# darcamo/pyphysim

Measured on AMD Instinct MI355X. Metric: Monte Carlo realizations/sec (whole node) + SER abs-error vs ref, higher is better.
Workload: dtype f64

## Files before the change

pyphysim_amd/csrc/capi.hip:

```cpp
#include <cmath>
#include <cstdarg>

#include "common.hpp"
#include "modem.hpp"

namespace mcle {

static thread_local char g_err[512] = "";

void set_error(const char* fmt, ...) {
    va_list ap;
    va_start(ap, fmt);
    vsnprintf(g_err, sizeof(g_err), fmt, ap);
    va_end(ap);
}

}

using namespace mcle;

int mcle_ctx::bind() const {
    MCLE_HIP(hipSetDevice(device));
    return MCLE_OK;
}
// ... 155 lines not shown
    if (ctx->ev1) (void)hipEventDestroy(ctx->ev1);
    if (ctx->ev_probe0) (void)hipEventDestroy(ctx->ev_probe0);
    if (ctx->ev_probe1) (void)hipEventDestroy(ctx->ev_probe1);
    if (ctx->own_stream && ctx->stream) (void)hipStreamDestroy(ctx->stream);
    delete ctx;
    return MCLE_OK;
}

int mcle_ctx_set_stream(mcle_ctx* ctx, void* hip_stream) {
    MCLE_REQUIRE(ctx != nullptr, "null context");
    MCLE_HIP(hipSetDevice(ctx->device));
    MCLE_HIP(hipStreamSynchronize(ctx->stream));
    if (ctx->own_stream && ctx->stream) MCLE_HIP(hipStreamDestroy(ctx->stream));
    if (hip_stream) {
        ctx->stream = (hipStream_t)hip_stream;
        ctx->own_stream = false;
    } else {
        MCLE_HIP(hipStreamCreateWithFlags(&ctx->stream, hipStreamNonBlocking));
        ctx->own_stream = true;
    }
    return MCLE_OK;
}

int mcle_ctx_get_stream(mcle_ctx* ctx, void** hip_stream) {
    MCLE_REQUIRE(ctx != nullptr && hip_stream != nullptr, "null argument");
    *hip_stream = (void*)ctx->stream;
    return MCLE_OK;
}

int mcle_ctx_set_option(mcle_ctx* ctx, int option, long long value) {
    MCLE_REQUIRE(ctx != nullptr, "null context");
    MCLE_REQUIRE(option >= 0 && option < MCLE_OPT_COUNT, "unknown option %d", option);
    bool ok = false;
    switch (option) {
        case MCLE_OPT_NO_MFMA: case MCLE_OPT_SINGLE_TDL: case MCLE_OPT_JAKES_DIRECT: case MCLE_OPT_F64_GENERIC: case MCLE_OPT_BD_RUNTIME_SOLVE: case MCLE_OPT_DEMOD_NOCERT: case MCLE_OPT_F32_MFMA: case MCLE_OPT_WALK_LEGACY: case MCLE_OPT_STAGED_GENERIC: case MCLE_OPT_CODEBOOK_NO_PACK: ok = value == 0 || value == 1; break;
        case MCLE_OPT_TDL_KERNEL: ok = value >= 0 && value <= 4; break;
#ifdef MCLE_EXPERIMENTS
        case MCLE_OPT_MIMO_TDL_KERNEL: ok = value >= 0 && value <= 255; break;
#else
        case MCLE_OPT_MIMO_TDL_KERNEL: ok = value >= 0 && value <= 2; break;
#endif
#ifdef MCLE_EXPERIMENTS
        case MCLE_OPT_F64_VARIANT: ok = value >= 0 && value <= 2047; break;
#else
        case MCLE_OPT_F64_VARIANT:
            MCLE_REQUIRE(value == 0, "option MCLE_OPT_F64_VARIANT: the timing-bound variants are compiled with -DMCLE_EXPERIMENTS only");
            ok = true;
            break;
#endif
        case MCLE_OPT_MFMA_VARIANT: ok = value == 0 || value == 36 || value == 32 || value == 30 || value == 21; break;
        case MCLE_OPT_GRID_OVERSUB: ok = value >= 0 && value <= 64; break;
        case MCLE_OPT_FLAT_WGS_PER_CU: ok = value >= 0 && value <= 4096; break;
        case MCLE_OPT_TDL_MFMA_WAVES: ok = value == 0 || value == 2 || value == 3 || value == 32; break;
        case MCLE_OPT_F64_THREADS: ok = value == 0 || (value >= 256 && value <= 266) || value == 512 || value == 1024; break;
    }
    MCLE_REQUIRE(ok, "option %d: value %lld out of range", option, value);
    ctx->opt[option] = value;
    return MCLE_OK;
}

int mcle_ctx_trim_scratch(mcle_ctx* ctx) {
    MCLE_REQUIRE(ctx != nullptr, "null context");
    MCLE_HIP(hipSetDevice(ctx->device));
    MCLE_HIP(hipStreamSynchronize(ctx->stream));
    if (ctx->d_scratch) MCLE_HIP(hipFree(ctx->d_scratch));
    ctx->d_scratch = nullptr;
    ctx->scratch_bytes = 0;
    return MCLE_OK;
}

int mcle_ctx_get_option(mcle_ctx* ctx, int option, long long* value) {
    MCLE_REQUIRE(ctx != nullptr && value != nullptr, "null argument");
    MCLE_REQUIRE(option >= 0 && option < MCLE_OPT_COUNT, "unknown option %d", option);
    *value = ctx->opt[option];
    return MCLE_OK;
}

int mcle_ctx_sync(mcle_ctx* ctx) {
    MCLE_REQUIRE(ctx != nullptr, "null context");
    MCLE_HIP(hipSetDevice(ctx->device));
    MCLE_HIP(hipStreamSynchronize(ctx->stream));
    return MCLE_OK;
}

int mcle_ctx_device_info(mcle_ctx* ctx, int* n_cu, int* lds_bytes, char* name, int name_len) {
    MCLE_REQUIRE(ctx != nullptr, "null context");
    if (n_cu) *n_cu = ctx->n_cu;
    if (lds_bytes) *lds_bytes = ctx->lds_bytes;
    if (name && name_len > 0) {
        std::strncpy(name, ctx->name.c_str(), name_len - 1);
        name[name_len - 1] = 0;
    }
    return MCLE_OK;
}

int mcle_ctx_last_kernel(mcle_ctx* ctx, char* name, int len) {
    MCLE_REQUIRE(ctx != nullptr && name != nullptr && len > 0, "null argument");
    std::strncpy(name, ctx->last_kernel, len - 1);
    name[len - 1] = 0;
    return MCLE_OK;
}

int mcle_malloc(mcle_ctx* ctx, size_t bytes, void** d_ptr) {
    MCLE_REQUIRE(ctx != nullptr && d_ptr != nullptr, "null argument");
    MCLE_HIP(hipSetDevice(ctx->device));
    *d_ptr = nullptr;
    if (bytes == 0) return MCLE_OK;
// ... 283 lines not shown
```

pyphysim_amd/csrc/pipeline_mimo_planar.hip:

```cpp
#include <type_traits>
#include <utility>

#include "fft.hpp"
#include "fft_r16.hpp"
#include "mimo.hpp"
#include "modem.hpp"
#include "philox.hpp"
#include "totals.hpp"
#include "pipe_common.hpp"
#include "mimo_planar_common.hpp"

namespace mcle {

template <typename T, int N, int NT, int NR, int AH, int WPS, int VAR = 0>
__global__ __launch_bounds__((N / 4) * (NR / AH), WPS) void k_run_mimo_ofdm_planar(MimoParams pp, ModemParams<T> mp, uint64_t seed,
                                                                     uint64_t first, uint64_t count,
                                                                     const cx<T>* __restrict__ g_tw,
                                                                     const cx<T>* __restrict__ g_recs,
                                                                     mcle_counters* counters,
                                                                     uint32_t* __restrict__ sym_out,
                                                                     uint32_t* __restrict__ bit_out) {
    using SH = F64Shape<N>;
    static_assert(NT >= 1 && NT <= NR && NR % AH == 0 && N >= 256, "geometry");
    constexpr int kRec = d64_rec<NT, NR>(), NB = SH::NB, N4 = SH::N4;
// ... 406 lines not shown
        hipLaunchKernelGGL((k_mimo_filters_planar<T, N, NT, NR>), dim3((unsigned)((n + 63) / 64)), dim3(64), 0, ctx->stream, pp, seed,
                           first + off, n, (cx<T>*)recs);
        MCLE_LAUNCH_CHECK();
        const unsigned grid = (unsigned)oversubscribed_grid(ctx, resident, n, flush_min_units(8, sizeof(T) == 4 ? 25600 : 12800, (uint64_t)N * NR), 16);
        hipLaunchKernelGGL(kern, dim3(grid), dim3(TB), lds, ctx->stream, pp, mp, seed, first + off, n,
                           (const cx<T>*)tw, (const cx<T>*)recs, d_counters, d_sym ? d_sym + off : nullptr,
                           d_bit ? d_bit + off : nullptr);
        MCLE_LAUNCH_CHECK();
    }
    return MCLE_OK;
}

#ifndef MCLE_PLANAR_F32_WPS_PLUS
#define MCLE_PLANAR_F32_WPS_PLUS 2
#endif
template <typename T> constexpr int planar_wps(int n, int nt, int nr, int w64) {
    if (sizeof(T) == 4 && w64 <= 3 && ((n == 256 && !(nt == 4 && nr == 4)) || (n == 512 && nr == 2))) return w64 + MCLE_PLANAR_F32_WPS_PLUS;
#ifndef MCLE_PLANAR_F64_256_WPS3
#define MCLE_PLANAR_F64_256_WPS3 0
#endif
    if (MCLE_PLANAR_F64_256_WPS3 && sizeof(T) == 8 && n == 256 && nr <= 3 && w64 == 2) return 3;
    return w64;
}

int run_mimo_ofdm_qw(mcle_ctx* ctx, const mcle_mimo_ofdm_cfg* cfg, uint64_t seed, uint64_t first, uint64_t count,
                     mcle_counters* d_counters, uint32_t* d_sym, uint32_t* d_bit);

int run_mimo_ofdm_fw(mcle_ctx* ctx, int dtype, const mcle_mimo_ofdm_cfg* cfg, uint64_t seed, uint64_t first, uint64_t count,
                     mcle_counters* d_counters, uint32_t* d_sym, uint32_t* d_bit);

int run_mimo_ofdm_pw(mcle_ctx* ctx, const mcle_mimo_ofdm_cfg* cfg, uint64_t seed, uint64_t first, uint64_t count,
                     mcle_counters* d_counters, uint32_t* d_sym, uint32_t* d_bit);

template <typename T>
static int run_mimo_ofdm_planar_t(mcle_ctx* ctx, const mcle_mimo_ofdm_cfg* cfg, uint64_t seed, uint64_t first, uint64_t count,
                                  mcle_counters* d_counters, uint32_t* d_sym, uint32_t* d_bit) {
    constexpr bool F64 = sizeof(T) == 8;
    const int n = cfg->fft_size, nt = cfg->nt, nr = cfg->nr;
#define MCLE_F64_GEOM(N_, NT_, NR_, AH_, WPS_)                                                                      \
    if (n == N_ && nt == NT_ && nr == NR_)                                                                          \
        return launch_mimo_ofdm_planar<T, N_, NT_, NR_, AH_, planar_wps<T>(N_, NT_, NR_, WPS_)>(ctx, cfg, seed, first, count, d_counters, d_sym, d_bit);
    if (n == 256 && nt == 4 && nr == 4) {
        {
            const long long thr = ctx->opt[MCLE_OPT_F64_THREADS];
            if (thr == 0 || thr == 260 || thr == 262) {
                const int rq = run_mimo_ofdm_fw(ctx, F64 ? MCLE_F64 : MCLE_F32, cfg, seed, first, count, d_counters, d_sym, d_bit);
                if (rq != MCLE_E_UNSUPPORTED) return rq;
            }
        }
    }
    if ((n == 512 || n == 2048) && nt == 4 && nr == 4) {
        if constexpr (F64) {
            const long long thr = ctx->opt[MCLE_OPT_F64_THREADS];
            if (thr == 0 || thr == 260 || thr == 262 || thr == 265 || thr == 266) {
                const int rq = run_mimo_ofdm_pw(ctx, cfg, seed, first, count, d_counters, d_sym, d_bit);
                if (rq != MCLE_E_UNSUPPORTED) return rq;
            }
        }
    }
    if (n == 1024 && nt == 4 && nr == 4) {
        if constexpr (F64) {
            {
                const long long thr = ctx->opt[MCLE_OPT_F64_THREADS];
                if (thr == 0 || thr == 263 || thr == 264 || thr == 265 || thr == 266) {
                    const int rq = run_mimo_ofdm_pw(ctx, cfg, seed, first, count, d_counters, d_sym, d_bit);
                    if (rq != MCLE_E_UNSUPPORTED) return rq;
                }
            }
            {
                const long long thr = ctx->opt[MCLE_OPT_F64_THREADS];
                if (thr == 0 || thr == 260 || thr == 262) {
                    const int rq = run_mimo_ofdm_qw(ctx, cfg, seed, first, count, d_counters, d_sym, d_bit);
                    if (rq != MCLE_E_UNSUPPORTED) return rq;
                }
            }
#ifdef MCLE_EXPERIMENTS
            switch ((int)ctx->opt[MCLE_OPT_F64_VARIANT]) {
                case 1: return launch_mimo_ofdm_planar<T, 1024, 4, 4, 2, 4, 1>(ctx, cfg, seed, first, count, d_counters, d_sym, d_bit);
                case 2: return launch_mimo_ofdm_planar<T, 1024, 4, 4, 2, 4, 2>(ctx, cfg, seed, first, count, d_counters, d_sym, d_bit);
                case 3: return launch_mimo_ofdm_planar<T, 1024, 4, 4, 2, 4, 3>(ctx, cfg, seed, first, count, d_counters, d_sym, d_bit);
                default: break;
            }
            switch ((int)ctx->opt[MCLE_OPT_F64_VARIANT]) {
#define MCLE_ABL(V_) case V_: return launch_mimo_ofdm_planar<T, 1024, 4, 4, 4, 2, 12 | V_>(ctx, cfg, seed, first, count, d_counters, d_sym, d_bit);
                MCLE_ABL(32) MCLE_ABL(64) MCLE_ABL(128) MCLE_ABL(256) MCLE_ABL(512) MCLE_ABL(1024) MCLE_ABL(2016) MCLE_ABL(1920) MCLE_ABL(384)
#undef MCLE_ABL
                default: break;
            }
#endif
            if (ctx->opt[MCLE_OPT_F64_THREADS] == 258)
                return launch_mimo_ofdm_planar<T, 1024, 4, 4, 4, 2, 28>(ctx, cfg, seed, first, count, d_counters, d_sym, d_bit);
        }
        if (ctx->opt[MCLE_OPT_F64_THREADS] == 256)
            return launch_mimo_ofdm_planar<T, 1024, 4, 4, 4, 2>(ctx, cfg, seed, first, count, d_counters, d_sym, d_bit);
        if (ctx->opt[MCLE_OPT_F64_THREADS] == 512)
            return launch_mimo_ofdm_planar<T, 1024, 4, 4, 2, 4>(ctx, cfg, seed, first, count, d_counters, d_sym, d_bit);
        if constexpr (!F64) {
            if (ctx->opt[MCLE_OPT_F64_THREADS] == 259)
                return launch_mimo_ofdm_planar<T, 1024, 4, 4, 4, 4, 12>(ctx, cfg, seed, first, count, d_counters, d_sym, d_bit);
            if (ctx->opt[MCLE_OPT_F64_THREADS] == 257)
                return launch_mimo_ofdm_planar<T, 1024, 4, 4, 4, 3, 4>(ctx, cfg, seed, first, count, d_counters, d_sym, d_bit);
            return launch_mimo_ofdm_planar<T, 1024, 4, 4, 4, 4, 4>(ctx, cfg, seed, first, count, d_counters, d_sym, d_bit);
        } else {
            if (ctx->opt[MCLE_OPT_F64_THREADS] == 257)
                return launch_mimo_ofdm_planar<T, 1024, 4, 4, 4, 2, 4>(ctx, cfg, seed, first, count, d_counters, d_sym, d_bit);
            return launch_mimo_ofdm_planar<T, 1024, 4, 4, 4, 2, 12>(ctx, cfg, seed, first, count, d_counters, d_sym, d_bit);
        }
    }
#define MCLE_F64_SIZE(N_, W2_, W4_)                                                                                  \
    MCLE_F64_GEOM(N_, 2, 2, 2, W2_) MCLE_F64_SIZE_REST(N_, W2_, W4_)
#define MCLE_F64_SIZE_REST(N_, W2_, W4_)                                                                             \
    MCLE_F64_GEOM(N_, 1, 2, 2, W2_)                                                                                  \
    MCLE_F64_GEOM(N_, 1, 3, 3, 2) MCLE_F64_GEOM(N_, 2, 3, 3, 2) MCLE_F64_GEOM(N_, 3, 3, 3, 2)                        \
    MCLE_F64_GEOM(N_, 1, 4, 2, W4_) MCLE_F64_GEOM(N_, 2, 4, 2, W4_) MCLE_F64_GEOM(N_, 3, 4, 2, W4_)
    MCLE_F64_SIZE_REST(256, 2, 3) MCLE_F64_GEOM(256, 4, 4, 2, 3)
    MCLE_F64_SIZE(512, 3, 3) MCLE_F64_GEOM(512, 4, 4, 2, 3)
    if (n == 1024 && nr == 4 && ctx->opt[MCLE_OPT_F64_THREADS] == 0) {
// ... 31 lines not shown
```

pyphysim_amd/csrc/pipeline_mimo_pw.hip:

```cpp
#include "mimo_planar_common.hpp"
#include "walk_f64.hpp"

namespace mcle {

constexpr int kPwPlane = 4 * 272;
__host__ __device__ __forceinline__ int pw_slot(int a, int e) { return a * 272 + e + (e >> 4); }
__host__ __device__ __forceinline__ int pw_mtime(int h, int c) { return (c & 3) * 64 + (c >> 2) * 16 + (h & 3) * 4 + (h >> 2); }
template <int NW> constexpr int pw_lab_stride() { return 16 * NW + 16; }
template <int NW> constexpr size_t pw_static_lds() {
    return (size_t)((kBmLdsDoubles + 1) & ~1) * sizeof(double) + (size_t)64 * pw_lab_stride<NW>() + 2 * (d64_rec<4, 4>() + 1) * sizeof(double2) +
           64 * sizeof(unsigned) + sizeof(WgTotals);
}

__device__ __forceinline__ void pw_row_swap(uint32_t& x, uint32_t& y) {
#if defined(__HIP_DEVICE_COMPILE__)
#if __has_builtin(__builtin_amdgcn_permlane16_swap)
    const auto s = __builtin_amdgcn_permlane16_swap(x, y, false, false);
    x = s[0];
    y = s[1];
#else
    const bool odd = (__lane_id() & 16) != 0;
    const uint32_t give = odd ? x : y, got = (uint32_t)__shfl_xor((int)give, 16);
    if (odd) x = got;
    else y = got;
// ... 56 lines not shown
#pragma unroll
                    for (int q = 0; q < 8; ++q) X[q] = mk<double>((double)(w0 + w1), 1.0);
                } else {
#pragma unroll
                    for (int q = 0; q < 4; ++q) {
                        X[q] = s_txtab[(w0 >> (8 * q)) & 0xFFu];
                        X[q + 4] = s_txtab[(w1 >> (8 * q)) & 0xFFu];
                    }
                }
                double2 A[4];
#pragma unroll
                for (int q = 0; q < 4; ++q) A[q] = (J & 1) ? csub(X[q], X[q + 4]) : cadd(X[q], X[q + 4]);
                const double2 B0 = cadd(A[0], rotJ(A[2])), B1 = cadd(A[1], rotJ(A[3]));
                double2 S;
                if constexpr (J == 0) S = cadd(B0, B1);
                else if constexpr (J == 2) S = mk<double>(B0.x - B1.y, B0.y + B1.x);
                else if constexpr (J == 4) S = csub(B0, B1);
                else if constexpr (J == 6) S = mk<double>(B0.x + B1.y, B0.y - B1.x);
                else {
                    constexpr double c = (J == 1 || J == 7) ? kH : -kH, sn = (J == 1 || J == 3) ? kH : -kH;
                    S = mk<double>(B0.x + (c * B1.x - sn * B1.y), B0.y + (sn * B1.x + c * B1.y));
                }
                if constexpr (J == 0) v[u] = S;
                else if (u == 0) v[u] = S;
                else v[u] = cmulc(S, g_tw[16 * J * u]);
            }
        }
    } else {
        static_assert(NW == 2, "first stage");
#pragma unroll
        for (int i = 0; i < 2; ++i) {
            const uint4 L = lab[i];
            const uint32_t wds[4] = {L.x, L.y, L.z, L.w};
#pragma unroll
            for (int uu = 0; uu < 8; ++uu) {
                const int u = 8 * i + uu;
                const uint32_t w = wds[uu >> 1] >> (16 * (uu & 1));
                double2 X0, X1;
                if constexpr (STUB) {
                    X0 = X1 = mk<double>((double)(w & 0xFFFFu), 1.0);
                } else {
                    X0 = s_txtab[w & 0xFFu];
                    X1 = s_txtab[(w >> 8) & 0xFFu];
                }
                const double2 S = J ? csub(X0, X1) : cadd(X0, X1);
                if constexpr (J == 0) v[u] = S;
                else if (u == 0) v[u] = S;
                else v[u] = cmulc(S, g_tw[16 * J * u]);
            }
        }
    }
}

template <int NW, int DEC, int WPS, bool TD = false, int ABL = 0, bool ROWS = !TD>
__global__ __launch_bounds__(64 * NW, WPS) void k_run_mimo_ofdm_pw(MimoParams pp, ModemParams<double> mp, uint64_t seed, uint64_t first,
                                                                   uint64_t count, const double2* __restrict__ g_tw,
                                                                   const double2* __restrict__ g_recs, mcle_counters* counters,
                                                                   uint32_t* __restrict__ sym_out, uint32_t* __restrict__ bit_out) {
    using T = double;
    constexpr int N = 256 * NW, NT = 4, NR = 4, kRec = d64_rec<NT, NR>(), TB = 64 * NW, UU = 16 / NW;
    constexpr int kLabStride = pw_lab_stride<NW>();
    static_assert(NW == 2 || NW == 4 || NW == 8, "wavefronts per realization");
    static_assert(!(TD && ROWS), "the time-domain form keeps the map wavefront = class");
    constexpr int kLogNW = NW == 2 ? 1 : NW == 4 ? 2 : 3;
    extern __shared__ __attribute__((aligned(16))) char pw_smem[];
    constexpr int kBm = (kBmLdsDoubles + 1) & ~1;
    __shared__ __attribute__((aligned(16))) double s_bm[kBm];
    __shared__ __attribute__((aligned(16))) unsigned char s_lab[64 * kLabStride];
    __shared__ __attribute__((aligned(16))) cx<T> s_rec[2 * (kRec + 1)];
    __shared__ unsigned s_part[64];
    __shared__ WgTotals totals;
    static_assert(sizeof(s_bm) + sizeof(s_lab) + sizeof(s_rec) + sizeof(s_part) + sizeof(totals) == pw_static_lds<NW>(), "launcher's LDS sum");
    T* s_R = reinterpret_cast<T*>(pw_smem);
    cx<T>* s_table = reinterpret_cast<cx<T>*>(s_R + NW * kPwPlane);
    cx<T>* s_txtab = s_table + ((mp.M + 1) & ~1);

    const int tid = threadIdx.x, lane = tid & 63;
    const int j = __builtin_amdgcn_readfirstlane(tid >> 6);
    const int pj = j & 1;
    const int cp = pp.cp;
    const int per_sym = N * NT;
    const uint64_t row = (uint64_t)pp.n_ofdm_sym * (N + cp);
    const T sigma = (T)sqrt(pp.noise_var);
    const T tx_scale = (T)(1.0 / sqrt((double)NT) / sqrt((double)(N + cp)));
    const T tab_scale = TD ? tx_scale : tx_scale * (T)N;
    const uint32_t mask = (uint32_t)(mp.M - 1);
    for (int m = tid; m < mp.M; m += TB) {
        const cx<T> c = mp.g_table[m];
        s_table[m] = c;
        s_txtab[m] = cscale(c, tab_scale);
    }
    if constexpr (ROWS) bm_tables_to_lds_pairs(s_bm, tid, TB);
    else bm_tables_to_lds(s_bm, tid, TB);
    if (tid == 0) wg_zero(totals);

    T* s_mine = s_R + j * kPwPlane;
    uint2* s_words_mine = reinterpret_cast<uint2*>(s_mine);
    uint64_t it = 0, rl_prev = 0;
    cx<T> rec_next = mk<T>(0, 0);
    if (tid < kRec && blockIdx.x < count) rec_next = g_recs[(uint64_t)blockIdx.x * kRec + tid];
    __syncthreads();
    for (uint64_t rl = blockIdx.x; rl < count; rl += gridDim.x, ++it) {
        const Rng rng(seed, first + rl);
        const int buf = (int)(it & 1);
        if (tid < kRec) {
            s_rec[buf * (kRec + 1) + tid] = rec_next;
            if (rl + gridDim.x < count) rec_next = g_recs[(rl + gridDim.x) * kRec + tid];
        }
        const cx<T>* s_H = s_rec + buf * (kRec + 1);
        const cx<T>* s_G = s_H + NT * NR;
        unsigned se = 0, be = 0;
        for (int os = 0; os < pp.n_ofdm_sym; ++os) {
            if (it > 0 || os > 0) __syncthreads();
            if constexpr (ROWS && !(ABL & 128)) __builtin_amdgcn_s_waitcnt(0xC07F);
            {
                const int t = opaque(tid);
                Words4 dw;
                if constexpr (ABL & 32) dw.w[0] = dw.w[1] = dw.w[2] = dw.w[3] = (uint32_t)t * 0x01010101u;
                else dw = rng.block(STREAM_DATA, (uint32_t)(((uint64_t)os * per_sym) >> 4) + (uint32_t)t);
                const int q = (t >> 6) ^ (NW / 2), u = (t & 63) >> 2;
#pragma unroll
                for (int s = 0; s < 4; ++s) {
                    const uint32_t w = dw.w[s] & (mask * 0x01010101u);
                    const int g = 4 * (t & 3) + s;
                    unsigned char* dst = s_lab + g * kLabStride + NW * u + q;
#pragma unroll
                    for (int a = 0; a < 4; ++a) dst[a * 16 * kLabStride] = (unsigned char)(w >> (8 * a));
                }
            }
            if constexpr (!ROWS) {
                const int ln = opaque(lane);
                const int r = ln >> 4, h = ln & 15;
                const uint64_t i00 = (uint64_t)r * row + (uint64_t)os * (N + cp) + cp + (j & ~1) + 32 * NW * pj + NW * (uint64_t)pw_mtime(h, 0);
                const uint32_t b0 = (uint32_t)(i00 >> 1);
                uint2* w_even = reinterpret_cast<uint2*>(s_R + (j & ~1) * kPwPlane) + (8 * pj) * 64 + ln;
                uint2* w_odd = reinterpret_cast<uint2*>(s_R + (j | 1) * kPwPlane) + (8 * pj) * 64 + ln;
#pragma unroll
                for (int cc = 0; cc < 8; ++cc) {
                    Words4 b;
                    if constexpr (ABL & 128) b.w[0] = b.w[1] = b.w[2] = b.w[3] = b0 + cc;
                    else b = rng.block(STREAM_NOISE, b0 + (uint32_t)(NW / 2) * (uint32_t)pw_mtime(0, cc));
                    w_even[cc * 64] = make_uint2(b.w[0], b.w[1]);
                    w_odd[cc * 64] = make_uint2(b.w[2], b.w[3]);
                }
            }
            auto account_prev = [&]() {
                if (tid == 0 && os == 0 && it > 0) {
                    const unsigned* qq = s_part + (buf ^ 1) * 32;
                    unsigned ts = 0, tb = 0;
#pragma unroll
                    for (int i = 0; i < NW; ++i) {
                        ts += qq[2 * i];
                        tb += qq[2 * i + 1];
                    }
                    wg_account(totals, ts, tb, s_rec[(buf ^ 1) * (kRec + 1) + 2 * NT * NR].x != 0.0, rl_prev, sym_out, bit_out);
                }
            };
            if constexpr (!ROWS) {
                __syncthreads();
                account_prev();
            }
            cx<T> v[16];
            if constexpr (TD) {
                const int ln = opaque(lane);
                const unsigned char* lab = s_lab + ln * kLabStride;
                if constexpr (NW == 4) {
// ... 81 lines not shown
                        pw_row_swap(b.w[1], b.w[3]);
                        v[cc] = mk<T>((T)b.w[0], sigma);
                        v[8 + cc] = mk<T>((T)b.w[2], sigma);
                    }
                } else {
                    BmFetched ft[8][2];
                    auto fetch = [&](int cc) {
                        Words4 b = rng.block(STREAM_NOISE, b0 + (uint32_t)(NW / 2) * (uint32_t)pw_mtime(0, cc));
                        pw_row_swap(b.w[0], b.w[2]);
                        pw_row_swap(b.w[1], b.w[3]);
                        ft[cc][0] = cn_fetch_lds_pairs(b.w[0], b.w[1], s_bm);
                        ft[cc][1] = cn_fetch_lds_pairs(b.w[2], b.w[3], s_bm);
                    };
                    fetch(0);
#pragma unroll
                    for (int cc = 0; cc < 8; ++cc) {
                        if (cc + 1 < 8) fetch(cc + 1);
                        __builtin_amdgcn_sched_barrier(0);
                        v[cc] = cn_finish(ft[cc][0], sigma);
                        v[8 + cc] = cn_finish(ft[cc][1], sigma);
                        __builtin_amdgcn_sched_barrier(0);
                    }
                }
            }
            if constexpr (TD) {
                const int ln = opaque(lane);
                const cx<T> hA = s_H[(ln & 3) * NT + (ln >> 4)];
                const T hre = hA.x, him = hA.y, nhim = -hA.y;
#pragma unroll
                for (int c = 0; c < 16; ++c) {
                    cx<T> z;
                    if constexpr (ABL & 128) z = mk<T>((T)nw[c].x, sigma);
                    else z = cn_words(nw[c].x, nw[c].y, sigma, s_bm);
                    if constexpr (ABL & 256) {
                        v[c] = cadd(v[c], z);
                    } else {
                        T yr = __builtin_amdgcn_mfma_f64_4x4x4f64(hre, v[c].x, z.x, 0, 0, 0);
                        T yi = __builtin_amdgcn_mfma_f64_4x4x4f64(him, v[c].x, z.y, 0, 0, 0);
                        yr = __builtin_amdgcn_mfma_f64_4x4x4f64(nhim, v[c].y, yr, 0, 0, 0);
                        yi = __builtin_amdgcn_mfma_f64_4x4x4f64(hre, v[c].y, yi, 0, 0, 0);
                        v[c] = mk<T>(yr, yi);
                    }
                }
            }
            if constexpr (!(ABL & 512)) {
                R16Tw64<T> none;
                r16_pass<T, false, true, 0, false, true, true, false, true>(nullptr, nullptr, 0, none, nullptr, 0, v, v);
            }
            {
                const int ln = opaque(lane);
                const int a = ln >> 4, g = ln & 15;
                const int wbase = pw_slot(a, g), rbase = pw_slot(a, 16 * g);
                T xr[16];
#pragma unroll
                for (int c = 0; c < 16; ++c) s_mine[rbase + c] = v[c].x;
                walk_wave_order();
#pragma unroll
                for (int u = 0; u < 16; ++u) xr[u] = s_mine[wbase + 17 * u];
                walk_wave_order();
#pragma unroll
                for (int c = 0; c < 16; ++c) s_mine[rbase + c] = v[c].y;
                walk_wave_order();
#pragma unroll
                for (int u = 0; u < 16; ++u) v[u] = mk<T>(xr[u], s_mine[wbase + 17 * u]);
            }
            if constexpr (!(ABL & 512)) {
                const int g = opaque(lane) & 15;
                R16Tw64<T> tw;
#pragma unroll
                for (int m = 1; m <= 3; ++m) {
                    tw.a1[m - 1] = g_tw[NW * g * m];
                    tw.a2[m - 1] = g_tw[4 * NW * g * m];
                }
                r16_pass<T, false, true, 0, false, true, true>(nullptr, nullptr, 0, tw, nullptr, 0, v, v);
            }
            T er[NW][UU], ei[NW][UU];
            constexpr bool kAhead = ROWS && ABL == 0;
            constexpr uint32_t kTwBytes = (uint32_t)sizeof(cx<T>);
            uint32_t kp0 = 0;
            static_assert(16 * kTwBytes * (NW - 1) * (UU - 1) < 4096, "the load's immediate offset");
            auto tw_at = [&](int m, int uu) {
                const char* lane_base = reinterpret_cast<const char*>(g_tw) + (size_t)(kTwBytes * (uint32_t)m * kp0);
                return *reinterpret_cast<const cx<T>*>(lane_base + 16 * (int)kTwBytes * m * uu);
            };
            cx<T> twb[2][NW - 1];
            uint4 lab_ahead = make_uint4(0, 0, 0, 0);
            cx<T> hA_ahead = mk<T>(0, 0), gA_ahead = mk<T>(0, 0);
            {
                const int ln = opaque(lane);
                const int r = ln >> 4, g = ln & 15;
                constexpr int kClass = ROWS ? 272 : kPwPlane;
                const int wpos = r * 272 + g + (ROWS ? 16 * (((4 * j + r) >> kLogNW) & 1) : 0);
                const int rpos = (ROWS ? NW * r * 272 + 16 * (r & 1) : r * 272) + g + 16 * UU * j;
                r16_wave_sync();
#pragma unroll
                for (int u = 0; u < 16; ++u) s_mine[wpos + 16 * u] = v[u].x;
                __syncthreads();
                if constexpr (ROWS) account_prev();
#pragma unroll
                for (int jj = 0; jj < NW; ++jj)
#pragma unroll
                    for (int uu = 0; uu < UU; ++uu) er[jj][uu] = s_R[jj * kClass + rpos + 16 * uu];
                __syncthreads();
#pragma unroll
                for (int u = 0; u < 16; ++u) s_mine[wpos + 16 * u] = v[u].y;
                if constexpr (kAhead) {
                    kp0 = (uint32_t)opaque((ln & 15) + 16 * UU * j);
#pragma unroll
                    for (int m = 1; m < NW; ++m) twb[0][m - 1] = tw_at(m, 0);
                    lab_ahead = *reinterpret_cast<const uint4*>(s_lab + ln * kLabStride + 16 * j);
                    hA_ahead = s_H[(ln & 3) * NT + (ln >> 4)];
                    gA_ahead = s_G[(ln & 3) * NR + (ln >> 4)];
                }
                __syncthreads();
#pragma unroll
                for (int jj = 0; jj < NW; ++jj)
#pragma unroll
                    for (int uu = 0; uu < UU; ++uu) ei[jj][uu] = s_R[jj * kClass + rpos + 16 * uu];
            }
            if constexpr (!(ABL & 1024)) {
                const int ln = opaque(lane);
                if constexpr (!kAhead) kp0 = (uint32_t)opaque((ln & 15) + 16 * UU * j);
                auto tw_of = [&](int m, int uu) {
                    if constexpr (kAhead) return twb[uu & 1][m - 1];
                    else return tw_at(m, uu);
                };
#pragma unroll
                for (int uu = 0; uu < UU; ++uu) {
                    if constexpr (kAhead) {
                        if (uu + 1 < UU) {
#pragma unroll
                            for (int m = 1; m < NW; ++m) twb[(uu + 1) & 1][m - 1] = tw_at(m, uu + 1);
                        }
                        __builtin_amdgcn_sched_barrier(0);
                    }
                    if constexpr (NW == 4) {
                        const cx<T> w1 = tw_of(1, uu), w2 = tw_of(2, uu), w3 = tw_of(3, uu);
                        const cx<T> u0 = mk<T>(er[0][uu], ei[0][uu]);
                        const cx<T> u1 = cmul(mk<T>(er[1][uu], ei[1][uu]), w1);
                        const cx<T> u2 = cmul(mk<T>(er[2][uu], ei[2][uu]), w2);
                        const cx<T> u3 = cmul(mk<T>(er[3][uu], ei[3][uu]), w3);
                        CxOps<T>::template bfly4<false>(u0, u1, u2, u3, v[4 * uu], v[4 * uu + 1], v[4 * uu + 2], v[4 * uu + 3]);
                    } else if constexpr (NW == 8) {
                        cx<T> x[8];
                        x[0] = mk<T>(er[0][uu], ei[0][uu]);
#pragma unroll
                        for (int jj = 1; jj < 8; ++jj) x[jj] = cmul(mk<T>(er[jj][uu], ei[jj][uu]), tw_of(jj, uu));
                        cx<T> E[4], O[4];
                        CxOps<T>::template bfly4<false>(x[0], x[2], x[4], x[6], E[0], E[1], E[2], E[3]);
                        CxOps<T>::template bfly4<false>(x[1], x[3], x[5], x[7], O[0], O[1], O[2], O[3]);
                        constexpr T kH = (T)0.70710678118654752440;
                        const cx<T> t0 = O[0];
                        const cx<T> t1 = mk<T>(kH * (O[1].x + O[1].y), kH * (O[1].y - O[1].x));
                        const cx<T> t2 = mk<T>(O[2].y, -O[2].x);
                        const cx<T> t3 = mk<T>(kH * (O[3].y - O[3].x), -kH * (O[3].x + O[3].y));
                        v[8 * uu + 0] = cadd(E[0], t0); v[8 * uu + 4] = csub(E[0], t0);
                        v[8 * uu + 1] = cadd(E[1], t1); v[8 * uu + 5] = csub(E[1], t1);
                        v[8 * uu + 2] = cadd(E[2], t2); v[8 * uu + 6] = csub(E[2], t2);
                        v[8 * uu + 3] = cadd(E[3], t3); v[8 * uu + 7] = csub(E[3], t3);
                    } else {
                        const cx<T> u0 = mk<T>(er[0][uu], ei[0][uu]);
                        const cx<T> u1 = cmul(mk<T>(er[1][uu], ei[1][uu]), tw_of(1, uu));
                        v[2 * uu] = cadd(u0, u1);
                        v[2 * uu + 1] = csub(u0, u1);
                    }
                }
            }
            {
                const int ln = opaque(lane);
                uint4 L;
                if constexpr (kAhead) L = lab_ahead;
                else L = *reinterpret_cast<const uint4*>(s_lab + ln * kLabStride + 16 * j);
                const uint32_t wds[4] = {L.x, L.y, L.z, L.w};
                if constexpr (!TD && !(ABL & 256)) {
                    cx<T> hA;
                    if constexpr (kAhead) hA = hA_ahead;
                    else hA = s_H[(ln & 3) * NT + (ln >> 4)];
                    const T hre = hA.x, him = hA.y, nhim = -hA.y;
#pragma unroll
                    for (int i = 0; i < 4; ++i) {
                        cx<T> X[4];
#pragma unroll
                        for (int jj = 0; jj < 4; ++jj) {
                            const uint32_t lb = (wds[i] >> (8 * jj)) & 0xFFu;
                            if constexpr (ABL & 32) X[jj] = mk<T>((T)lb, 1.0);
                            else X[jj] = s_txtab[lb];
                        }
                        T yr[4], yi[4];
#pragma unroll
                        for (int jj = 0; jj < 4; ++jj) {
                            yr[jj] = __builtin_amdgcn_mfma_f64_4x4x4f64(hre, X[jj].x, v[4 * i + jj].x, 0, 0, 0);
                            yi[jj] = __builtin_amdgcn_mfma_f64_4x4x4f64(him, X[jj].x, v[4 * i + jj].y, 0, 0, 0);
                        }
#pragma unroll
                        for (int jj = 0; jj < 4; ++jj) {
                            yr[jj] = __builtin_amdgcn_mfma_f64_4x4x4f64(nhim, X[jj].y, yr[jj], 0, 0, 0);
                            yi[jj] = __builtin_amdgcn_mfma_f64_4x4x4f64(hre, X[jj].y, yi[jj], 0, 0, 0);
                            v[4 * i + jj] = mk<T>(yr[jj], yi[jj]);
                        }
                    }
                }
                if constexpr (!(ABL & 1024)) {
                cx<T> gA;
                if constexpr (kAhead) gA = gA_ahead;
                else gA = s_G[(ln & 3) * NR + (ln >> 4)];
                const T gre = gA.x, gim = gA.y, ngim = -gA.y;
#pragma unroll
                for (int i = 0; i < 4; ++i) {
                    cx<T> e[4];
#pragma unroll
                    for (int jj = 0; jj < 4; ++jj) {
                        const int u = 4 * i + jj;
                        T xr = __builtin_amdgcn_mfma_f64_4x4x4f64(gre, v[u].x, 0.0, 0, 0, 0);
                        T xi = __builtin_amdgcn_mfma_f64_4x4x4f64(gim, v[u].x, 0.0, 0, 0, 0);
                        xr = __builtin_amdgcn_mfma_f64_4x4x4f64(ngim, v[u].y, xr, 0, 0, 0);
                        xi = __builtin_amdgcn_mfma_f64_4x4x4f64(gre, v[u].y, xi, 0, 0, 0);
                        e[jj] = mk<T>(xr, xi);
                    }
                    if constexpr (DEC == WDEC_SLICER || DEC == WDEC_QAM_CERT) {
                        walk_qam_count4<DEC == WDEC_QAM_CERT>(mp, s_table, e, wds[i], se, be);
                    } else {
                        int tx[4];
#pragma unroll
                        for (int jj = 0; jj < 4; ++jj) tx[jj] = (int)((wds[i] >> (8 * jj)) & 0xFFu);
                        walk_decide<DEC, 4>(mp, s_table, nullptr, e, tx, se, be);
                    }
                }
                } else {
                    T keep = er[0][0] + ei[NW - 1][UU - 1];
                    if constexpr (!TD) {
#pragma unroll
                        for (int u = 0; u < 16; ++u) keep += v[u].x + v[u].y;
                    }
                    se += (unsigned)(keep == 0.5) + (wds[0] == 0x12345u);
                }
            }
        }
        se = wave_sum_u32(se);
        be = wave_sum_u32(be);
        if (lane == 0) {
            s_part[buf * 32 + 2 * j] = se;
            s_part[buf * 32 + 2 * j + 1] = be;
        }
        rl_prev = rl;
    }
    __syncthreads();
    if (tid == 0) {
        if (it > 0) {
            const int buf = (int)((it - 1) & 1);
            const unsigned* qq = s_part + buf * 32;
            unsigned ts = 0, tb = 0;
#pragma unroll
            for (int i = 0; i < NW; ++i) {
                ts += qq[2 * i];
                tb += qq[2 * i + 1];
            }
            wg_account(totals, ts, tb, s_rec[buf * (kRec + 1) + 2 * NT * NR].x != 0.0, rl_prev, sym_out, bit_out);
        }
        wg_flush(totals, counters, (unsigned long long)per_sym * pp.n_ofdm_sym, (unsigned long long)per_sym * pp.n_ofdm_sym * mp.bits);
    }
}

template <int NW, int WPS, bool TD = false, int ABL = 0, bool ROWS = !TD>
static int launch_mimo_ofdm_pw(mcle_ctx* ctx, const mcle_mimo_ofdm_cfg* cfg, uint64_t seed, uint64_t first, uint64_t count,
                               mcle_counters* d_counters, uint32_t* d_sym, uint32_t* d_bit) {
    using T = double;
    constexpr int N = 256 * NW, NT = 4, NR = 4, kRec = d64_rec<NT, NR>();
    int rc;
    void* tw = nullptr;
    if ((rc = ctx->get_twiddles(N, MCLE_F64, &tw))) return rc;
    MimoParams pp{cfg->cp_size, cfg->num_used, cfg->n_ofdm_sym, cfg->mmse, cfg->noise_var};
    ModemParams<T> mp = pipe_modem<T>(ctx, cfg->demod_method);
    const int dec = walk_dec_kind(ctx, mp);
    mp.grid.G = 0;
    const size_t tab_len = ((size_t)mp.M + 1) & ~(size_t)1;
    const size_t dyn = (size_t)NW * kPwPlane * sizeof(T) + 2 * tab_len * sizeof(cx<T>);
    const size_t lds = dyn + pw_static_lds<NW>();
    MCLE_REQUIRE(lds + 512 <= (size_t)160 * 1024, "part-wave MIMO-OFDM kernel: %zu B of LDS do not fit", lds);
    auto kern = k_run_mimo_ofdm_pw<NW, WDEC_SLICER, WPS, TD, ABL, ROWS>;
    switch (dec) {
        case WDEC_QAM_CERT: kern = k_run_mimo_ofdm_pw<NW, WDEC_QAM_CERT, WPS, TD, ABL, ROWS>; break;
        case WDEC_QUAD_CERT: kern = k_run_mimo_ofdm_pw<NW, WDEC_QUAD_CERT, WPS, TD, ABL, ROWS>; break;
        case WDEC_AXIS4_CERT: kern = k_run_mimo_ofdm_pw<NW, WDEC_AXIS4_CERT, WPS, TD, ABL, ROWS>; break;
        default: break;
    }
    MCLE_HIP(hipFuncSetAttribute((const void*)kern, hipFuncAttributeMaxDynamicSharedMemorySize, (int)dyn));
    int per_cu = (int)((size_t)160 * 1024 / (lds + 512));
    if (per_cu < 1) per_cu = 1;
    const int by_waves = WPS * 4 / NW;
    if (per_cu > by_waves) per_cu = by_waves;
    const uint64_t resident = (uint64_t)ctx->n_cu * per_cu;
    ctx->set_kernel("mimo_ofdm_pw<%d>/%s%s%s", NW, TD ? "time" : "freq", WPS == (NW == 8 ? 2 : 3) ? "" : "/w2", !TD && !ROWS ? "/a" : "");
    const uint64_t kSlice = 1ull << 20;
    const uint64_t slice = count < kSlice ? count : kSlice;
    void* recs = nullptr;
    if ((rc = ctx->scratch((size_t)slice * kRec * sizeof(cx<T>), &recs))) return rc;
    for (uint64_t off = 0; off < count; off += slice) {
        const uint64_t n = count - off < slice ? count - off : slice;
        hipLaunchKernelGGL((k_mimo_filters_planar<T, N, NT, NR>), dim3((unsigned)((n + 63) / 64)), dim3(64), 0, ctx->stream, pp, seed,
                           first + off, n, (cx<T>*)recs);
        MCLE_LAUNCH_CHECK();
        const unsigned grid = (unsigned)oversubscribed_grid(ctx, resident, n, 8, NW == 4 ? 32 : 16);
        hipLaunchKernelGGL(kern, dim3(grid), dim3(64 * NW), dyn, ctx->stream, pp, mp, seed, first + off, n, (const cx<T>*)tw,
                           (const cx<T>*)recs, d_counters, d_sym ? d_sym + off : nullptr, d_bit ? d_bit + off : nullptr);
        MCLE_LAUNCH_CHECK();
    }
    return MCLE_OK;
}

int run_mimo_ofdm_pw(mcle_ctx* ctx, const mcle_mimo_ofdm_cfg* cfg, uint64_t seed, uint64_t first, uint64_t count,
                     mcle_counters* d_counters, uint32_t* d_sym, uint32_t* d_bit) {
    if (!((cfg->fft_size == 512 || cfg->fft_size == 1024 || cfg->fft_size == 2048) && cfg->nt == 4 && cfg->nr == 4 && cfg->num_used == cfg->fft_size &&
          (cfg->cp_size & 1) == 0))
        return MCLE_E_UNSUPPORTED;
    if (ctx->M > 256) return MCLE_E_UNSUPPORTED;
    {
        ModemParams<double> mp = pipe_modem<double>(ctx, cfg->demod_method);
        if (walk_dec_kind(ctx, mp) == WDEC_GENERIC) return MCLE_E_UNSUPPORTED;
    }
    const bool two = ctx->opt[MCLE_OPT_F64_THREADS] == 262 || ctx->opt[MCLE_OPT_F64_THREADS] == 264;
    const bool td = ctx->opt[MCLE_OPT_F64_THREADS] == 265;
    if (ctx->opt[MCLE_OPT_F64_THREADS] == 266) {
        if (cfg->fft_size == 2048) return launch_mimo_ofdm_pw<8, 2, false, 0, false>(ctx, cfg, seed, first, count, d_counters, d_sym, d_bit);
        if (cfg->fft_size == 512) return launch_mimo_ofdm_pw<2, 3, false, 0, false>(ctx, cfg, seed, first, count, d_counters, d_sym, d_bit);
        return launch_mimo_ofdm_pw<4, 3, false, 0, false>(ctx, cfg, seed, first, count, d_counters, d_sym, d_bit);
    }
    if (cfg->fft_size == 2048) {
        return td ? launch_mimo_ofdm_pw<8, 2, true>(ctx, cfg, seed, first, count, d_counters, d_sym, d_bit)
                  : launch_mimo_ofdm_pw<8, 2>(ctx, cfg, seed, first, count, d_counters, d_sym, d_bit);
    }
#ifdef MCLE_EXPERIMENTS
#define MCLE_PW_ABL(NW_, V_)                                                                                          \
    case V_:                                                                                                          \
        return td ? launch_mimo_ofdm_pw<NW_, 3, true, V_>(ctx, cfg, seed, first, count, d_counters, d_sym, d_bit)     \
                  : launch_mimo_ofdm_pw<NW_, 3, false, V_>(ctx, cfg, seed, first, count, d_counters, d_sym, d_bit);
#define MCLE_PW_ABLS(NW_)                                                                                             \
    switch ((int)ctx->opt[MCLE_OPT_F64_VARIANT]) {                                                                    \
        MCLE_PW_ABL(NW_, 32) MCLE_PW_ABL(NW_, 64) MCLE_PW_ABL(NW_, 128) MCLE_PW_ABL(NW_, 256) MCLE_PW_ABL(NW_, 512)   \
        MCLE_PW_ABL(NW_, 1024) MCLE_PW_ABL(NW_, 2016)                                                                 \
        default: break;                                                                                               \
    }
#else
#define MCLE_PW_ABLS(NW_)
#endif
    if (cfg->fft_size == 512) {
        MCLE_PW_ABLS(2)
        if (td) return launch_mimo_ofdm_pw<2, 3, true>(ctx, cfg, seed, first, count, d_counters, d_sym, d_bit);
        return two ? launch_mimo_ofdm_pw<2, 2>(ctx, cfg, seed, first, count, d_counters, d_sym, d_bit)
                   : launch_mimo_ofdm_pw<2, 3>(ctx, cfg, seed, first, count, d_counters, d_sym, d_bit);
    }
    MCLE_PW_ABLS(4)
#undef MCLE_PW_ABLS
#ifdef MCLE_EXPERIMENTS
#undef MCLE_PW_ABL
#endif
    if (td) return launch_mimo_ofdm_pw<4, 3, true>(ctx, cfg, seed, first, count, d_counters, d_sym, d_bit);
    return two ? launch_mimo_ofdm_pw<4, 2>(ctx, cfg, seed, first, count, d_counters, d_sym, d_bit)
               : launch_mimo_ofdm_pw<4, 3>(ctx, cfg, seed, first, count, d_counters, d_sym, d_bit);
}

}
```

Baseline: 48.68 million.

## Exchange FFT data between wavefronts in complex halves through LDS

The inter-wavefront exchange before the final radix stage of the part-wave f64 MIMO-OFDM kernel now stores and reloads whole complex values in two halves, using a shared LDS buffer with two barriers. The twiddle, label and channel look-ahead loads are placed between those barriers. The aim is to replace the separate real and imaginary plane exchange with fewer, wider LDS accesses and to overlap the prefetches with the exchange, at the cost of an extra barrier. This form becomes the default for the 1024 and 2048 sizes, while 512 keeps the old form. New option values 267 and 268 select it explicitly, and a compile-time flag moves the earlier barrier later.

```diff
diff --git a/pyphysim_amd/csrc/capi.hip b/pyphysim_amd/csrc/capi.hip
--- a/pyphysim_amd/csrc/capi.hip
+++ b/pyphysim_amd/csrc/capi.hip
@@ -231,7 +231,7 @@
         case MCLE_OPT_GRID_OVERSUB: ok = value >= 0 && value <= 64; break;
         case MCLE_OPT_FLAT_WGS_PER_CU: ok = value >= 0 && value <= 4096; break;
         case MCLE_OPT_TDL_MFMA_WAVES: ok = value == 0 || value == 2 || value == 3 || value == 32; break;
-        case MCLE_OPT_F64_THREADS: ok = value == 0 || (value >= 256 && value <= 266) || value == 512 || value == 1024; break;
+        case MCLE_OPT_F64_THREADS: ok = value == 0 || (value >= 256 && value <= 268) || value == 512 || value == 1024; break;
     }
     MCLE_REQUIRE(ok, "option %d: value %lld out of range", option, value);
     ctx->opt[option] = value;
diff --git a/pyphysim_amd/csrc/pipeline_mimo_planar.hip b/pyphysim_amd/csrc/pipeline_mimo_planar.hip
--- a/pyphysim_amd/csrc/pipeline_mimo_planar.hip
+++ b/pyphysim_amd/csrc/pipeline_mimo_planar.hip
@@ -482,7 +482,7 @@
     if ((n == 512 || n == 2048) && nt == 4 && nr == 4) {
         if constexpr (F64) {
             const long long thr = ctx->opt[MCLE_OPT_F64_THREADS];
-            if (thr == 0 || thr == 260 || thr == 262 || thr == 265 || thr == 266) {
+            if (thr == 0 || thr == 260 || thr == 262 || thr == 265 || thr == 266 || thr == 267 || thr == 268) {
                 const int rq = run_mimo_ofdm_pw(ctx, cfg, seed, first, count, d_counters, d_sym, d_bit);
                 if (rq != MCLE_E_UNSUPPORTED) return rq;
             }
@@ -492,7 +492,7 @@
         if constexpr (F64) {
             {
                 const long long thr = ctx->opt[MCLE_OPT_F64_THREADS];
-                if (thr == 0 || thr == 263 || thr == 264 || thr == 265 || thr == 266) {
+                if (thr == 0 || thr == 263 || thr == 264 || thr == 265 || thr == 266 || thr == 267 || thr == 268) {
                     const int rq = run_mimo_ofdm_pw(ctx, cfg, seed, first, count, d_counters, d_sym, d_bit);
                     if (rq != MCLE_E_UNSUPPORTED) return rq;
                 }
diff --git a/pyphysim_amd/csrc/pipeline_mimo_pw.hip b/pyphysim_amd/csrc/pipeline_mimo_pw.hip
--- a/pyphysim_amd/csrc/pipeline_mimo_pw.hip
+++ b/pyphysim_amd/csrc/pipeline_mimo_pw.hip
@@ -132,7 +132,7 @@
     }
 }
 
-template <int NW, int DEC, int WPS, bool TD = false, int ABL = 0, bool ROWS = !TD>
+template <int NW, int DEC, int WPS, bool TD = false, int ABL = 0, bool ROWS = !TD, bool XCH = ROWS && !TD>
 __global__ __launch_bounds__(64 * NW, WPS) void k_run_mimo_ofdm_pw(MimoParams pp, ModemParams<double> mp, uint64_t seed, uint64_t first,
                                                                    uint64_t count, const double2* __restrict__ g_tw,
                                                                    const double2* __restrict__ g_recs, mcle_counters* counters,
@@ -142,6 +142,13 @@
     constexpr int kLabStride = pw_lab_stride<NW>();
     static_assert(NW == 2 || NW == 4 || NW == 8, "wavefronts per realization");
     static_assert(!(TD && ROWS), "the time-domain form keeps the map wavefront = class");
+    static_assert(!XCH || (ROWS && ABL == 0), "the exchange in complex halves belongs to the default form by lane row");
+    constexpr bool kAhead = ROWS && ABL == 0;
+#ifdef MCLE_PW_LATE_B5
+    constexpr bool kLateB5 = XCH && kAhead;
+#else
+    constexpr bool kLateB5 = false;
+#endif
     constexpr int kLogNW = NW == 2 ? 1 : NW == 4 ? 2 : 3;
     extern __shared__ __attribute__((aligned(16))) char pw_smem[];
     constexpr int kBm = (kBmLdsDoubles + 1) & ~1;
@@ -191,7 +198,9 @@
         const cx<T>* s_G = s_H + NT * NR;
         unsigned se = 0, be = 0;
         for (int os = 0; os < pp.n_ofdm_sym; ++os) {
-            if (it > 0 || os > 0) __syncthreads();
+            if constexpr (!kLateB5) {
+                if (it > 0 || os > 0) __syncthreads();
+            }
             if constexpr (ROWS && !(ABL & 128)) __builtin_amdgcn_s_waitcnt(0xC07F);
             {
                 const int t = opaque(tid);
@@ -379,6 +388,11 @@
                 const int a = ln >> 4, g = ln & 15;
                 const int wbase = pw_slot(a, g), rbase = pw_slot(a, 16 * g);
                 T xr[16];
+                if constexpr (kLateB5) {
+#pragma unroll
+                    for (int c = 0; c < 16; ++c) asm volatile("" : "+v"(v[c].x), "+v"(v[c].y));
+                    if (it > 0 || os > 0) __syncthreads();
+                }
 #pragma unroll
                 for (int c = 0; c < 16; ++c) s_mine[rbase + c] = v[c].x;
                 walk_wave_order();
@@ -402,7 +416,7 @@
                 r16_pass<T, false, true, 0, false, true, true>(nullptr, nullptr, 0, tw, nullptr, 0, v, v);
             }
             T er[NW][UU], ei[NW][UU];
-            constexpr bool kAhead = ROWS && ABL == 0;
+            cx<T> ez[NW][UU];
             constexpr uint32_t kTwBytes = (uint32_t)sizeof(cx<T>);
             uint32_t kp0 = 0;
             static_assert(16 * kTwBytes * (NW - 1) * (UU - 1) < 4096, "the load's immediate offset");
@@ -413,7 +427,47 @@
             cx<T> twb[2][NW - 1];
             uint4 lab_ahead = make_uint4(0, 0, 0, 0);
             cx<T> hA_ahead = mk<T>(0, 0), gA_ahead = mk<T>(0, 0);
-            {
+            if constexpr (XCH) {
+                const int ln = opaque(lane);
+                const int r = ln >> 4, g = ln & 15;
+                constexpr int UH = UU / 2, kSl = 272 / 2;
+                cx<T>* s_X = reinterpret_cast<cx<T>*>(s_R);
+                const int wA = (4 * j + r) * kSl + g;
+                const int rA = NW * r * kSl + g + 16 * UH * j;
+                const int rB = NW == 2 ? (4 * (r & 1) + j) * kSl + g + 16 * UH * (r >> 1) : j * kSl + g + 16 * UH * (NW / 4) * r;
+                r16_wave_sync();
+#pragma unroll
+                for (int u = 0; u < 16; ++u) asm volatile("" : "+v"(v[u].x));
+                account_prev();
+#pragma unroll
+                for (int u = 0; u < 16; ++u) asm volatile("" : "+v"(v[u].y));
+#pragma unroll
+                for (int jw = 0; jw < NW; ++jw)
+#pragma unroll
+                    for (int uu = 0; uu < UH; ++uu) s_X[wA + 16 * (UH * jw + uu)] = v[UU * jw + uu];
+                __syncthreads();
+#pragma unroll
+                for (int jj = 0; jj < NW; ++jj)
+#pragma unroll
+                    for (int uu = 0; uu < UH; ++uu) ez[jj][uu] = s_X[rA + jj * kSl + 16 * uu];
+#pragma unroll
+                for (int jw = 0; jw < NW; ++jw)
+#pragma unroll
+                    for (int uu = UH; uu < UU; ++uu) s_X[rA + jw * kSl + 16 * (uu - UH)] = v[UU * jw + uu];
+                kp0 = (uint32_t)opaque((ln & 15) + 16 * UU * j);
+#pragma unroll
+                for (int m = 1; m < NW; ++m) twb[0][m - 1] = tw_at(m, 0);
+                lab_ahead = *reinterpret_cast<const uint4*>(s_lab + ln * kLabStride + 16 * j);
+                hA_ahead = s_H[(ln & 3) * NT + (ln >> 4)];
+                gA_ahead = s_G[(ln & 3) * NR + (ln >> 4)];
+                __syncthreads();
+#pragma unroll
+                for (int jj = 0; jj < NW; ++jj) {
+                    const int off = NW == 2 ? 2 * jj * kSl : (jj & 3) * NW * kSl + 16 * UH * (jj >> 2);
+#pragma unroll
+                    for (int uu = UH; uu < UU; ++uu) ez[jj][uu] = s_X[rB + off + 16 * (uu - UH)];
+                }
+            } else {
                 const int ln = opaque(lane);
                 const int r = ln >> 4, g = ln & 15;
                 constexpr int kClass = ROWS ? 272 : kPwPlane;
@@ -448,6 +502,10 @@
             if constexpr (!(ABL & 1024)) {
                 const int ln = opaque(lane);
                 if constexpr (!kAhead) kp0 = (uint32_t)opaque((ln & 15) + 16 * UU * j);
+                auto ex = [&](int jj, int uu) {
+                    if constexpr (XCH) return ez[jj][uu];
+                    else return mk<T>(er[jj][uu], ei[jj][uu]);
+                };
                 auto tw_of = [&](int m, int uu) {
                     if constexpr (kAhead) return twb[uu & 1][m - 1];
                     else return tw_at(m, uu);
@@ -463,16 +521,16 @@
                     }
                     if constexpr (NW == 4) {
                         const cx<T> w1 = tw_of(1, uu), w2 = tw_of(2, uu), w3 = tw_of(3, uu);
-                        const cx<T> u0 = mk<T>(er[0][uu], ei[0][uu]);
-                        const cx<T> u1 = cmul(mk<T>(er[1][uu], ei[1][uu]), w1);
-                        const cx<T> u2 = cmul(mk<T>(er[2][uu], ei[2][uu]), w2);
-                        const cx<T> u3 = cmul(mk<T>(er[3][uu], ei[3][uu]), w3);
+                        const cx<T> u0 = ex(0, uu);
+                        const cx<T> u1 = cmul(ex(1, uu), w1);
+                        const cx<T> u2 = cmul(ex(2, uu), w2);
+                        const cx<T> u3 = cmul(ex(3, uu), w3);
                         CxOps<T>::template bfly4<false>(u0, u1, u2, u3, v[4 * uu], v[4 * uu + 1], v[4 * uu + 2], v[4 * uu + 3]);
                     } else if constexpr (NW == 8) {
                         cx<T> x[8];
-                        x[0] = mk<T>(er[0][uu], ei[0][uu]);
-#pragma unroll
-                        for (int jj = 1; jj < 8; ++jj) x[jj] = cmul(mk<T>(er[jj][uu], ei[jj][uu]), tw_of(jj, uu));
+                        x[0] = ex(0, uu);
+#pragma unroll
+                        for (int jj = 1; jj < 8; ++jj) x[jj] = cmul(ex(jj, uu), tw_of(jj, uu));
                         cx<T> E[4], O[4];
                         CxOps<T>::template bfly4<false>(x[0], x[2], x[4], x[6], E[0], E[1], E[2], E[3]);
                         CxOps<T>::template bfly4<false>(x[1], x[3], x[5], x[7], O[0], O[1], O[2], O[3]);
@@ -486,8 +544,8 @@
                         v[8 * uu + 2] = cadd(E[2], t2); v[8 * uu + 6] = csub(E[2], t2);
                         v[8 * uu + 3] = cadd(E[3], t3); v[8 * uu + 7] = csub(E[3], t3);
                     } else {
-                        const cx<T> u0 = mk<T>(er[0][uu], ei[0][uu]);
-                        const cx<T> u1 = cmul(mk<T>(er[1][uu], ei[1][uu]), tw_of(1, uu));
+                        const cx<T> u0 = ex(0, uu);
+                        const cx<T> u1 = cmul(ex(1, uu), tw_of(1, uu));
                         v[2 * uu] = cadd(u0, u1);
                         v[2 * uu + 1] = csub(u0, u1);
                     }
@@ -588,7 +646,7 @@
     }
 }
 
-template <int NW, int WPS, bool TD = false, int ABL = 0, bool ROWS = !TD>
+template <int NW, int WPS, bool TD = false, int ABL = 0, bool ROWS = !TD, bool XCH = ROWS && ABL == 0>
 static int launch_mimo_ofdm_pw(mcle_ctx* ctx, const mcle_mimo_ofdm_cfg* cfg, uint64_t seed, uint64_t first, uint64_t count,
                                mcle_counters* d_counters, uint32_t* d_sym, uint32_t* d_bit) {
     using T = double;
@@ -604,11 +662,11 @@
     const size_t dyn = (size_t)NW * kPwPlane * sizeof(T) + 2 * tab_len * sizeof(cx<T>);
     const size_t lds = dyn + pw_static_lds<NW>();
     MCLE_REQUIRE(lds + 512 <= (size_t)160 * 1024, "part-wave MIMO-OFDM kernel: %zu B of LDS do not fit", lds);
-    auto kern = k_run_mimo_ofdm_pw<NW, WDEC_SLICER, WPS, TD, ABL, ROWS>;
+    auto kern = k_run_mimo_ofdm_pw<NW, WDEC_SLICER, WPS, TD, ABL, ROWS, XCH>;
     switch (dec) {
-        case WDEC_QAM_CERT: kern = k_run_mimo_ofdm_pw<NW, WDEC_QAM_CERT, WPS, TD, ABL, ROWS>; break;
-        case WDEC_QUAD_CERT: kern = k_run_mimo_ofdm_pw<NW, WDEC_QUAD_CERT, WPS, TD, ABL, ROWS>; break;
-        case WDEC_AXIS4_CERT: kern = k_run_mimo_ofdm_pw<NW, WDEC_AXIS4_CERT, WPS, TD, ABL, ROWS>; break;
+        case WDEC_QAM_CERT: kern = k_run_mimo_ofdm_pw<NW, WDEC_QAM_CERT, WPS, TD, ABL, ROWS, XCH>; break;
+        case WDEC_QUAD_CERT: kern = k_run_mimo_ofdm_pw<NW, WDEC_QUAD_CERT, WPS, TD, ABL, ROWS, XCH>; break;
+        case WDEC_AXIS4_CERT: kern = k_run_mimo_ofdm_pw<NW, WDEC_AXIS4_CERT, WPS, TD, ABL, ROWS, XCH>; break;
         default: break;
     }
     MCLE_HIP(hipFuncSetAttribute((const void*)kern, hipFuncAttributeMaxDynamicSharedMemorySize, (int)dyn));
@@ -617,7 +675,10 @@
     const int by_waves = WPS * 4 / NW;
     if (per_cu > by_waves) per_cu = by_waves;
     const uint64_t resident = (uint64_t)ctx->n_cu * per_cu;
-    ctx->set_kernel("mimo_ofdm_pw<%d>/%s%s%s", NW, TD ? "time" : "freq", WPS == (NW == 8 ? 2 : 3) ? "" : "/w2", !TD && !ROWS ? "/a" : "");
+    const long long asked = ctx->opt[MCLE_OPT_F64_THREADS];
+    static_assert(XCH ? ROWS && ABL == 0 : true, "the exchange in complex halves: default form by lane row only");
+    ctx->set_kernel("mimo_ofdm_pw<%d>/%s%s%s", NW, TD ? "time" : "freq", WPS == (NW == 8 ? 2 : 3) ? "" : "/w2",
+                    !TD && !ROWS ? "/a" : asked == 267 ? "/x" : asked == 268 ? "/h" : "");
     const uint64_t kSlice = 1ull << 20;
     const uint64_t slice = count < kSlice ? count : kSlice;
     void* recs = nullptr;
@@ -652,6 +713,16 @@
         if (cfg->fft_size == 512) return launch_mimo_ofdm_pw<2, 3, false, 0, false>(ctx, cfg, seed, first, count, d_counters, d_sym, d_bit);
         return launch_mimo_ofdm_pw<4, 3, false, 0, false>(ctx, cfg, seed, first, count, d_counters, d_sym, d_bit);
     }
+    if (ctx->opt[MCLE_OPT_F64_THREADS] == 268) {
+        if (cfg->fft_size == 2048) return launch_mimo_ofdm_pw<8, 2, false, 0, true, true>(ctx, cfg, seed, first, count, d_counters, d_sym, d_bit);
+        if (cfg->fft_size == 512) return launch_mimo_ofdm_pw<2, 3, false, 0, true, true>(ctx, cfg, seed, first, count, d_counters, d_sym, d_bit);
+        return launch_mimo_ofdm_pw<4, 3, false, 0, true, true>(ctx, cfg, seed, first, count, d_counters, d_sym, d_bit);
+    }
+    if (ctx->opt[MCLE_OPT_F64_THREADS] == 267) {
+        if (cfg->fft_size == 2048) return launch_mimo_ofdm_pw<8, 2, false, 0, true, false>(ctx, cfg, seed, first, count, d_counters, d_sym, d_bit);
+        if (cfg->fft_size == 512) return launch_mimo_ofdm_pw<2, 3, false, 0, true, false>(ctx, cfg, seed, first, count, d_counters, d_sym, d_bit);
+        return launch_mimo_ofdm_pw<4, 3, false, 0, true, false>(ctx, cfg, seed, first, count, d_counters, d_sym, d_bit);
+    }
     if (cfg->fft_size == 2048) {
         return td ? launch_mimo_ofdm_pw<8, 2, true>(ctx, cfg, seed, first, count, d_counters, d_sym, d_bit)
                   : launch_mimo_ofdm_pw<8, 2>(ctx, cfg, seed, first, count, d_counters, d_sym, d_bit);
@@ -673,8 +744,8 @@
     if (cfg->fft_size == 512) {
         MCLE_PW_ABLS(2)
         if (td) return launch_mimo_ofdm_pw<2, 3, true>(ctx, cfg, seed, first, count, d_counters, d_sym, d_bit);
-        return two ? launch_mimo_ofdm_pw<2, 2>(ctx, cfg, seed, first, count, d_counters, d_sym, d_bit)
-                   : launch_mimo_ofdm_pw<2, 3>(ctx, cfg, seed, first, count, d_counters, d_sym, d_bit);
+        return two ? launch_mimo_ofdm_pw<2, 2, false, 0, true, false>(ctx, cfg, seed, first, count, d_counters, d_sym, d_bit)
+                   : launch_mimo_ofdm_pw<2, 3, false, 0, true, false>(ctx, cfg, seed, first, count, d_counters, d_sym, d_bit);
     }
     MCLE_PW_ABLS(4)
 #undef MCLE_PW_ABLS
```

Measured after the change: 49.27 million, median of 6. +1.2%, better.
